# weiyithu/PV-RAFT

Hardware: AMD Instinct MI355X
Metric: train_pairs_per_sec (higher is better)
Workload: dtype bf16; 1 GPU; model=PV-RAFT (RSF stage 1), global_batch=2, points=8192, gru_iters=8, truncate_k=512, parallelism=dp1, hipgraph=True

## Files before the change

### pvraft_amd/csrc/bindings.cpp

```cpp
#include <torch/extension.h>
#include <ATen/hip/HIPContext.h>
#include <hip/hip_runtime.h>

#include <map>
#include <string>
#include <utility>

void launch_knn_graph(const float*, int*, int, int, int, hipStream_t);
void launch_knn_csr(const int*, int*, int*, int*, int*, int*, unsigned char*,
                    int, int, int, hipStream_t);
void launch_knn_interp(const float*, const float*, const float*, float*, int*,
                       float*, int, int, int, int, int, float, hipStream_t);
int knn_interp_tile_pts();
void launch_chamfer_fwd(const float*, const float*, const float*, float*, int*,
                        float*, int*, float*, int, int, int, int, int,
                        hipStream_t);
void launch_chamfer_bwd(const float*, const float*, const float*, const int*,
                        const int*, const float*, float*, int, int, int, int,
                        hipStream_t);
int chamfer_fwd_blocks(int, int, int);
int chamfer_tile_pts();
void launch_flow_smooth_fwd(const float*, const int*, float*, int, int, int,
                            int, hipStream_t);
void launch_flow_smooth_bwd(const float*, const int*, const int*, const int*,
// ... 1006 lines not shown
                                            std::vector<torch::Tensor> dbs) {
  const int n = (int)dys.size();
  TORCH_CHECK(n >= 1 && n <= 4095, "1..4095 jobs");
  TORCH_CHECK((int)xs.size() == n && (int)dws.size() == n && (int)dbs.size() == n);
  std::vector<PwWgradJob> jobs(n);
  long base_blocks = 0;
  const int TILE = 64;
  for (int j = 0; j < n; ++j) {
    auto& dy = dys[j];
    auto& x = xs[j];
    auto& dw = dws[j];
    TORCH_CHECK(dy.is_cuda() && dy.is_contiguous() && dy.dim() == 3 &&
                dy.scalar_type() == torch::kBFloat16, "dy must be (B,Co,S) bf16");
    TORCH_CHECK(x.is_cuda() && x.is_contiguous() && x.dim() == 3 &&
                x.scalar_type() == torch::kBFloat16, "x must be (B,Ci,S) bf16");
    TORCH_CHECK(dy.size(0) == x.size(0) && dy.size(2) == x.size(2), "dy/x mismatch");
    const bool dw_block = dw.dim() == 2 && !dw.is_contiguous();
    TORCH_CHECK(dw.is_cuda() && dw.scalar_type() == torch::kFloat32 &&
                (dw_block ? (dw.stride(1) == 1 && dw.stride(0) >= dw.size(1))
                          : dw.is_contiguous()),
                "dw must be fp32, contiguous or a row-contiguous block");
    const int Co = dy.size(1), Ci = x.size(1);
    TORCH_CHECK(dw.numel() == (long)Co * Ci &&
                (!dw_block || (dw.size(0) == Co && dw.size(1) == Ci)),
                "dw shape mismatch");
    const int ldw = dw_block ? (int)dw.stride(0) : Ci;
    TORCH_CHECK(Co <= 16 * TILE && Ci <= 16 * TILE, "Co/Ci too large for 4-bit tile index");
    float* dbias = nullptr;
    if (dbs[j].defined() && dbs[j].numel() > 0) {
      TORCH_CHECK(dbs[j].is_cuda() && dbs[j].is_contiguous() &&
                  dbs[j].scalar_type() == torch::kFloat32 && dbs[j].numel() == Co);
      dbias = dbs[j].data_ptr<float>();
    }
    jobs[j] = PwWgradJob{dy.data_ptr(), x.data_ptr(), dw.data_ptr<float>(),
                         dbias, Co, Ci, (int)dy.size(0), 1, dy.size(2), ldw,
                         0};
    base_blocks += (long)((Co + TILE - 1) / TILE) * ((Ci + TILE - 1) / TILE) *
                   dy.size(0);
  }
  (void)base_blocks;
  for (int j = 0; j < n; ++j) {
    long sc = (jobs[j].S + 3071) / 3072;
    if (sc < 1) sc = 1;
    if ((long)jobs[j].B * sc > 4095) sc = 4095 / jobs[j].B;
    jobs[j].schunks = (int)sc;
  }
  std::vector<unsigned int> map;
  map.reserve(4096);
  for (int j = 0; j < n; ++j) {
    const int to = (jobs[j].Co + TILE - 1) / TILE;
    const int ti = (jobs[j].Ci + TILE - 1) / TILE;
    const int bzs = jobs[j].B * jobs[j].schunks;
    for (int bz = 0; bz < bzs; ++bz)
      for (int a = 0; a < to; ++a)
        for (int b = 0; b < ti; ++b)
          map.push_back(((unsigned)j << 20) | ((unsigned)bz << 8) |
                        ((unsigned)a << 4) | (unsigned)b);
  }
  const long jbytes = (long)n * sizeof(PwWgradJob);
  const long mbytes = (long)map.size() * sizeof(unsigned int);
  std::vector<unsigned char> blob(jbytes + mbytes);
  memcpy(blob.data(), jobs.data(), jbytes);
  memcpy(blob.data() + jbytes, map.data(), mbytes);
  auto dev = torch::empty({jbytes + mbytes}, dys[0].options().dtype(torch::kUInt8));
  launch_desc_fill(dev.data_ptr(), blob.data(), jbytes + mbytes, stream());
  launch_pw_wgrad_batched(dev.data_ptr(),
                          (const unsigned int*)((char*)dev.data_ptr() + jbytes),
                          (int)map.size(), stream());
  return {dev};
}

torch::Tensor batched_transpose(torch::Tensor x) {
  TORCH_CHECK(x.is_cuda() && x.dim() == 3, "x must be 3-D GPU");
  TORCH_CHECK(x.stride(2) == 1 && x.stride(1) == x.size(2),
              "rows must be contiguous");
  const bool bf16 = x.scalar_type() == torch::kBFloat16;
  TORCH_CHECK(bf16 || x.scalar_type() == torch::kFloat32, "fp32/bf16 only");
  const int B = x.size(0);
  const long R = x.size(1), C = x.size(2);
  auto out = torch::empty({B, C, R}, x.options());
  launch_transpose(x.data_ptr(), out.data_ptr(), x.stride(0), B, R, C, bf16,
                   stream());
  return out;
}

std::vector<torch::Tensor> pv_corr_fused_fwd(torch::Tensor corr,
                                             torch::Tensor xyz,
                                             torch::Tensor coords,
                                             double base_scale,
                                             int64_t num_levels, int64_t k) {
  check_f32(corr, "corr");
  check_f32(xyz, "xyz");
  check_f32(coords, "coords");
  const int B = corr.size(0), N = corr.size(1), K = corr.size(2);
  TORCH_CHECK(K <= 512 && num_levels >= 1 && num_levels <= 4 && k >= 1 && k <= 64 && k <= K);
  auto vox = torch::empty({B, num_levels * 27, N}, corr.options());
  auto knn = torch::empty({B, 4, k, N}, corr.options());
  auto idx = torch::empty({B, N, k}, corr.options().dtype(torch::kInt32));
  launch_pv_corr_fused_fwd(corr.data_ptr<float>(), xyz.data_ptr<float>(),
                           coords.data_ptr<float>(), vox.data_ptr<float>(),
                           knn.data_ptr<float>(), idx.data_ptr<int>(), B, N, K,
                           (int)num_levels, (int)k, (float)base_scale, stream());
  return {vox, knn, idx};
}

torch::Tensor pv_corr_fused_bwd(torch::Tensor g_vox, torch::Tensor g_knn,
                                torch::Tensor xyz, torch::Tensor coords,
                                torch::Tensor knn_idx, int64_t num_levels,
                                int64_t k, double base_scale) {
  check_f32(g_vox, "g_vox");
  check_f32(g_knn, "g_knn");
  const int B = xyz.size(0), N = xyz.size(1), K = xyz.size(2);
  auto gcorr = torch::empty({B, N, K}, g_vox.options());
  launch_pv_corr_fused_bwd(g_vox.data_ptr<float>(), g_knn.data_ptr<float>(),
                           xyz.data_ptr<float>(), coords.data_ptr<float>(),
                           knn_idx.data_ptr<int>(), gcorr.data_ptr<float>(), B,
                           N, K, (int)num_levels, (int)k, (float)base_scale,
                           stream());
  return gcorr;
}

void launch_corr_topk(const void*, const void*, float*, float*, int*, float*,
                      int*, int*, int, int, int, int, int, float,
                      hipStream_t);

std::vector<torch::Tensor> corr_topk(torch::Tensor f1t, torch::Tensor f2t,
                                     int64_t K) {
  TORCH_CHECK(f1t.is_cuda() && f1t.is_contiguous() && f1t.dim() == 3 &&
              f1t.scalar_type() == torch::kBFloat16, "f1t must be (B,N,C) bf16");
  TORCH_CHECK(f2t.is_cuda() && f2t.is_contiguous() && f2t.dim() == 3 &&
              f2t.scalar_type() == torch::kBFloat16, "f2t must be (B,M,C) bf16");
  const int B = f1t.size(0), N = f1t.size(1), C = f1t.size(2);
  const int M = f2t.size(1);
  TORCH_CHECK(f2t.size(0) == B && f2t.size(2) == C, "f1t/f2t mismatch");
  TORCH_CHECK(C % 32 == 0 && C <= 256, "need C % 32 == 0, C <= 256");
  TORCH_CHECK(K >= 1 && K <= M && K <= 1024, "need 1 <= K <= min(M, 1024)");
  auto fopt = f1t.options().dtype(torch::kFloat32);
  auto iopt = f1t.options().dtype(torch::kInt32);
  const long R = (long)B * N;
  auto thr = torch::empty({R, 2}, fopt);
  auto out_v = torch::empty({B, (long)N, K}, fopt);
  auto out_i = torch::empty({B, (long)N, K}, iopt);
  auto band_v = torch::empty({R, 704}, fopt);
  auto band_i = torch::empty({R, 704}, iopt);
  auto cnt = zeros_fast({R, 2}, iopt);
  launch_corr_topk(f1t.data_ptr(), f2t.data_ptr(), thr.data_ptr<float>(),
                   out_v.data_ptr<float>(), out_i.data_ptr<int>(),
                   band_v.data_ptr<float>(), band_i.data_ptr<int>(),
                   cnt.data_ptr<int>(), B, N, M, C, (int)K,
                   1.0f / sqrtf((float)C), stream());
  return {out_v, out_i};
}

std::vector<torch::Tensor> topk_rows(torch::Tensor vals, int64_t K) {
  check_f32(vals, "vals");
  TORCH_CHECK(vals.dim() == 2, "vals must be (R, M)");
  const long R = vals.size(0);
  const int M = vals.size(1);
  TORCH_CHECK(M <= 8192, "topk_rows supports M <= 8192");
  TORCH_CHECK(K >= 1 && K <= M, "need 1 <= K <= M");
  auto out_v = torch::empty({R, K}, vals.options());
  auto out_i = torch::empty({R, K}, vals.options().dtype(torch::kInt32));
  launch_topk_rows(vals.data_ptr<float>(), out_v.data_ptr<float>(),
                   out_i.data_ptr<int>(), R, M, (int)K, stream());
  return {out_v, out_i};
}

namespace {

void check_gru(const torch::Tensor& t, const torch::Tensor& like,
               const char* name) {
  TORCH_CHECK(t.is_cuda() && t.is_contiguous(), name,
              " must be a contiguous GPU tensor");
  TORCH_CHECK(t.scalar_type() == like.scalar_type(), name,
              " dtype mismatch in fused GRU gates");
}

}

std::vector<torch::Tensor> gru_zr_fwd(torch::Tensor pre, torch::Tensor h) {
  TORCH_CHECK(pre.is_cuda() && pre.is_contiguous() && h.is_contiguous());
  TORCH_CHECK(pre.dim() == 3 && h.dim() == 3 && pre.size(0) == h.size(0) &&
              pre.size(1) == 2 * h.size(1) && pre.size(2) == h.size(2));
  const bool bf16 = pre.scalar_type() == torch::kBFloat16;
  TORCH_CHECK(bf16 || pre.scalar_type() == torch::kFloat32);
  check_gru(h, pre, "h");
  auto z = torch::empty_like(h), r = torch::empty_like(h),
       rh = torch::empty_like(h);
  launch_gru_zr_fwd(pre.data_ptr(), h.data_ptr(), z.data_ptr(), r.data_ptr(),
                    rh.data_ptr(), h.size(0), (long)h.size(1) * h.size(2),
                    bf16, stream());
  return {z, r, rh};
}

std::vector<torch::Tensor> gru_zr_bwd(torch::Tensor dz, torch::Tensor drh,
                                      torch::Tensor z, torch::Tensor r,
                                      torch::Tensor h) {
  const bool bf16 = z.scalar_type() == torch::kBFloat16;
  for (auto* t : {&dz, &drh, &r, &h}) check_gru(*t, z, "gru_zr_bwd input");
  auto dpre = torch::empty({h.size(0), 2 * h.size(1), h.size(2)}, h.options());
  auto dh = torch::empty_like(h);
  launch_gru_zr_bwd(dz.data_ptr(), drh.data_ptr(), z.data_ptr(), r.data_ptr(),
                    h.data_ptr(), dpre.data_ptr(), dh.data_ptr(), h.size(0),
                    (long)h.size(1) * h.size(2), bf16, stream());
  return {dpre, dh};
}

std::vector<torch::Tensor> gru_q_fwd(torch::Tensor pre, torch::Tensor z,
                                     torch::Tensor h) {
  const bool bf16 = pre.scalar_type() == torch::kBFloat16;
  TORCH_CHECK(bf16 || pre.scalar_type() == torch::kFloat32);
  for (auto* t : {&pre, &z, &h}) check_gru(*t, pre, "gru_q_fwd input");
  auto q = torch::empty_like(h), hnew = torch::empty_like(h);
  launch_gru_q_fwd(pre.data_ptr(), z.data_ptr(), h.data_ptr(), q.data_ptr(),
                   hnew.data_ptr(), h.size(0), (long)h.size(1) * h.size(2),
                   bf16, stream());
  return {q, hnew};
}

std::vector<torch::Tensor> gru_q_bwd(torch::Tensor dhnew, torch::Tensor q,
                                     torch::Tensor z, torch::Tensor h) {
  const bool bf16 = q.scalar_type() == torch::kBFloat16;
  for (auto* t : {&dhnew, &z, &h}) check_gru(*t, q, "gru_q_bwd input");
  auto dpre = torch::empty_like(h), dz = torch::empty_like(h),
       dh = torch::empty_like(h);
  launch_gru_q_bwd(dhnew.data_ptr(), q.data_ptr(), z.data_ptr(), h.data_ptr(),
                   dpre.data_ptr(), dz.data_ptr(), dh.data_ptr(), h.size(0),
                   (long)h.size(1) * h.size(2), bf16, stream());
  return {dpre, dz, dh};
}

std::vector<torch::Tensor> seq_loss_fwd(std::vector<torch::Tensor> flows,
                                        torch::Tensor gt, torch::Tensor mask,
                                        double gamma) {
  const int T = (int)flows.size();
  TORCH_CHECK(T >= 1 && T <= 32, "seq_loss supports 1..32 flows");
  check_f32(gt, "gt");
  check_f32(mask, "mask");
  const long BN = gt.numel() / 3;
  TORCH_CHECK(mask.numel() == BN, "mask/gt shape mismatch");
  const float* ptrs[32];
  for (int t = 0; t < T; ++t) {
    check_f32(flows[t], "flow");
    TORCH_CHECK(flows[t].numel() == BN * 3, "flow shape mismatch");
    ptrs[t] = flows[t].data_ptr<float>();
  }
  auto fopt = gt.options();
  static torch::Tensor* ws_p = new torch::Tensor();
  torch::Tensor& ws = *ws_p;
  if (!ws.defined()) ws = torch::zeros({33}, fopt);
  auto loss = torch::empty({}, fopt);
  auto denom = torch::empty({}, fopt);
  launch_seq_loss_fwd(ptrs, gt.data_ptr<float>(), mask.data_ptr<float>(),
                      ws.data_ptr<float>(), loss.data_ptr<float>(),
                      denom.data_ptr<float>(), BN, T, 1, (float)gamma,
                      stream());
  return {loss, denom};
}

std::vector<torch::Tensor> seq_loss_bwd(std::vector<torch::Tensor> flows,
                                        torch::Tensor gt, torch::Tensor mask,
                                        torch::Tensor dloss,
                                        torch::Tensor denom, double gamma) {
  const int T = (int)flows.size();
  TORCH_CHECK(T >= 1 && T <= 32);
  const long BN = gt.numel() / 3;
  const float* ptrs[32];
  float* gptrs[32];
  std::vector<torch::Tensor> grads;
  grads.reserve(T);
  for (int t = 0; t < T; ++t) {
    ptrs[t] = flows[t].data_ptr<float>();
    grads.push_back(torch::empty_like(flows[t]));
    gptrs[t] = grads[t].data_ptr<float>();
  }
  launch_seq_loss_bwd(ptrs, gptrs, gt.data_ptr<float>(),
                      mask.data_ptr<float>(), dloss.data_ptr<float>(),
                      denom.data_ptr<float>(), BN, T, 1, (float)gamma,
                      stream());
  return grads;
}

static void check_i32(const torch::Tensor& t, const char* name) {
  TORCH_CHECK(t.is_cuda() && t.is_contiguous() && t.scalar_type() == torch::kInt32,
              name, " must be a contiguous int32 GPU tensor");
}

static void chamfer_check(const torch::Tensor& pc1, const torch::Tensor& pc2,
                          int64_t T) {
  check_f32(pc1, "pc1");
  check_f32(pc2, "pc2");
  TORCH_CHECK(pc1.dim() == 3 && pc1.size(2) == 3, "pc1 must be (B,N,3)");
  TORCH_CHECK(pc2.dim() == 3 && pc2.size(2) == 3, "pc2 must be (B,M,3)");
  TORCH_CHECK(pc2.device() == pc1.device(), "chamfer inputs must share a device");
  const int64_t B = pc1.size(0), N = pc1.size(1), M = pc2.size(1);
  TORCH_CHECK(pc2.size(0) == B, "chamfer batch mismatch");
  TORCH_CHECK(T >= 1 && T <= 32, "chamfer supports 1..32 flows");
  TORCH_CHECK(B >= 1 && B <= 65535 && N >= 1 && M >= 1,
              "chamfer requires 1 <= B <= 65535, N, M >= 1");
  TORCH_CHECK(N < (1L << 31) - 256 && M < (1L << 31) - 256,
              "chamfer sizes exceed 32-bit point indexing");
}

std::vector<torch::Tensor> chamfer_fwd(torch::Tensor pc1, torch::Tensor flows,
                                       torch::Tensor pc2) {
  check_f32(flows, "flows");
// ... 206 lines not shown
  TORCH_CHECK(M >= 1 && M <= 256, "cluster_points requires 1 <= max_objects <= 256");
  TORCH_CHECK(min_points >= 3, "cluster_points requires min_points >= 3");
  TORCH_CHECK(eps >= 0.0 && flow_eps >= 0.0, "cluster_points requires eps, flow_eps >= 0");
  TORCH_CHECK(mask.is_cuda() && mask.is_contiguous() &&
                  mask.scalar_type() == torch::kBool && mask.dim() == 2 &&
                  mask.size(0) == B && mask.size(1) == N &&
                  mask.device() == xyz.device(),
              "mask must be contiguous bool (B,N) on the device of xyz");
  auto iopt = xyz.options().dtype(torch::kInt32);
  auto ws = torch::empty({5, B, N}, iopt);
  auto status = torch::empty({B}, iopt);
  auto labels = torch::empty({B, N}, iopt);
  auto count = torch::empty({B, M}, iopt);
  auto nobj = torch::empty({B}, iopt);
  launch_cluster_points(
      xyz.data_ptr<float>(), flow.data_ptr<float>(),
      reinterpret_cast<const unsigned char*>(mask.data_ptr<bool>()),
      ws.data_ptr<int>(), status.data_ptr<int>(), labels.data_ptr<int>(),
      count.data_ptr<int>(), nobj.data_ptr<int>(), (int)B, (int)N, (int)M,
      (float)eps, (float)flow_eps, (int)std::min<int64_t>(min_points, INT32_MAX),
      stream());
  return {labels, count, nobj};
}

std::vector<torch::Tensor> plane_fit(torch::Tensor xyz,
                                     c10::optional<torch::Tensor> mask,
                                     double thresh, double thresh2, double cos2,
                                     double upx, double upy, double upz,
                                     int64_t H, int64_t refine_iters,
                                     int64_t seed) {
  check_f32(xyz, "xyz");
  TORCH_CHECK(xyz.dim() == 3 && xyz.size(2) == 3, "xyz must be (B,N,3)");
  const int64_t B = xyz.size(0), N = xyz.size(1);
  TORCH_CHECK(B >= 1 && B <= 65535 && N >= 1, "plane_fit requires 1 <= B <= 65535, N >= 1");
  TORCH_CHECK(N < (1L << 30), "plane_fit sizes exceed 32-bit point indexing");
  TORCH_CHECK(H >= 1 && H <= 4096, "plane_fit requires 1 <= hypotheses <= 4096");
  TORCH_CHECK(refine_iters <= 16, "plane_fit requires refine_iters <= 16");
  TORCH_CHECK(thresh > 0.0 && thresh2 > 0.0, "plane_fit requires thresh > 0");
  const unsigned char* mp = nullptr;
  if (mask.has_value()) {
    const torch::Tensor& m = *mask;
    TORCH_CHECK(m.is_cuda() && m.is_contiguous() &&
                    m.scalar_type() == torch::kBool && m.dim() == 2 &&
                    m.size(0) == B && m.size(1) == N &&
                    m.device() == xyz.device(),
                "mask must be contiguous bool (B,N) on the device of xyz");
    mp = reinterpret_cast<const unsigned char*>(m.data_ptr<bool>());
  }
  auto iopt = xyz.options().dtype(torch::kInt32);
  auto bopt = xyz.options().dtype(torch::kBool);
  auto idx = torch::empty({B, H, 3}, iopt);
  auto cnt = torch::empty({B, H}, iopt);
  auto rec = torch::empty({B, H, 8}, xyz.options());
  launch_plane_hypotheses(xyz.data_ptr<float>(), mp, idx.data_ptr<int>(),
                          rec.data_ptr<float>(), cnt.data_ptr<int>(), (int)B,
                          (int)N, (int)H, (unsigned)(seed & 0xffffffffL),
                          (float)upx, (float)upy, (float)upz, (float)cos2,
                          (float)thresh2, stream());
  if (refine_iters < 0) return {idx, cnt};
  auto normal = torch::empty({B, 3}, xyz.options());
  auto offset = torch::empty({B}, xyz.options());
  auto height = torch::empty({B, N}, xyz.options());
  auto ground = torch::empty({B, N}, bopt);
  auto inlier = torch::empty({B, N}, bopt);
  auto count = torch::empty({B}, iopt);
  auto best = torch::empty({B}, iopt);
  auto rounds = torch::empty({B}, iopt);
  auto ok = torch::empty({B}, bopt);
  auto plane64 = torch::empty({B, 8}, xyz.options().dtype(torch::kFloat64));
  launch_plane_refine(
      xyz.data_ptr<float>(), mp, rec.data_ptr<float>(), cnt.data_ptr<int>(),
      normal.data_ptr<float>(), offset.data_ptr<float>(),
      height.data_ptr<float>(),
      reinterpret_cast<unsigned char*>(ground.data_ptr<bool>()),
      reinterpret_cast<unsigned char*>(inlier.data_ptr<bool>()),
      count.data_ptr<int>(), best.data_ptr<int>(), rounds.data_ptr<int>(),
      reinterpret_cast<unsigned char*>(ok.data_ptr<bool>()),
      plane64.data_ptr<double>(), (int)B, (int)N, (int)H, (int)refine_iters,
      thresh, (float)upx, (float)upy, (float)upz, (float)cos2, stream());
  return {normal, offset, height, ground, inlier, count, best, rounds, ok};
}

std::vector<torch::Tensor> voxel_sample(torch::Tensor xyz,
                                        c10::optional<torch::Tensor> mask,
                                        int64_t m, double inv, int64_t levels,
                                        int64_t seed) {
  check_f32(xyz, "xyz");
  TORCH_CHECK(xyz.dim() == 3 && xyz.size(2) == 3, "xyz must be (B,N,3)");
  const int64_t B = xyz.size(0), N = xyz.size(1);
  TORCH_CHECK(B >= 1 && B <= 65535 && N >= 1, "voxel_sample requires 1 <= B <= 65535, N >= 1");
  TORCH_CHECK(N < (1L << 27), "voxel_sample requires N < 2^27");
  TORCH_CHECK(m >= 1, "voxel_sample requires m >= 1");
  TORCH_CHECK(levels >= 1 && levels <= 16, "voxel_sample requires 1 <= levels <= 16");
  TORCH_CHECK(inv > 0.0 && std::isfinite(inv), "voxel_sample requires a finite 1 / voxel > 0");
  const unsigned char* mp = nullptr;
  if (mask.has_value()) {
    const torch::Tensor& k = *mask;
    TORCH_CHECK(k.is_cuda() && k.is_contiguous() &&
                    k.scalar_type() == torch::kBool && k.dim() == 2 &&
                    k.size(0) == B && k.size(1) == N &&
                    k.device() == xyz.device(),
                "mask must be contiguous bool (B,N) on the device of xyz");
    mp = reinterpret_cast<const unsigned char*>(k.data_ptr<bool>());
  }
  int64_t T = 2;
  while (T < 2 * N) T <<= 1;
  const int64_t nblk = (N + voxel_sample_block() - 1) / voxel_sample_block();
  auto iopt = xyz.options().dtype(torch::kInt32);
  auto lopt = xyz.options().dtype(torch::kInt64);
  auto tab = torch::empty({6, B, T}, lopt);
  auto key0 = torch::empty({B, N}, lopt);
  auto slots = torch::empty({2, B, N}, iopt);
  auto sel = torch::empty({B, N}, xyz.options().dtype(torch::kUInt8));
  auto bsum = torch::empty({B, nblk}, iopt);
  auto meta = torch::empty({B, (int64_t)voxel_sample_meta()}, iopt);
  auto idx = torch::empty({B, m}, lopt);
  auto count = torch::empty({B}, iopt);
  auto rank = torch::empty({B, N}, iopt);
  auto occ = torch::empty({B, levels}, iopt);
  launch_voxel_sample(
      xyz.data_ptr<float>(), mp,
      reinterpret_cast<unsigned long long*>(tab.data_ptr<int64_t>()),
      reinterpret_cast<unsigned long long*>(key0.data_ptr<int64_t>()),
      slots.data_ptr<int>(), sel.data_ptr<uint8_t>(), bsum.data_ptr<int>(),
      meta.data_ptr<int>(), reinterpret_cast<long*>(idx.data_ptr<int64_t>()),
      count.data_ptr<int>(), rank.data_ptr<int>(), occ.data_ptr<int>(), (int)B,
      (int)N, (int)T, (long)m, (int)levels, (float)inv,
      (unsigned)(seed & 0xffffffffL), stream());
  return {idx, count, rank, occ};
}

PYBIND11_MODULE(TORCH_EXTENSION_NAME, m) {
  m.def("voxel_sample", &voxel_sample);
  m.attr("VOXEL_SAMPLE_BLOCK") = voxel_sample_block();
  m.attr("VOXEL_SAMPLE_SCAN") = voxel_sample_scan();
  m.def("plane_fit", &plane_fit);
  m.attr("PLANE_SCORE_TILE") = plane_score_tile();
  m.attr("PLANE_SCORE_BLOCK") = plane_score_block();
  m.attr("PLANE_REFINE_BLOCK") = plane_refine_block();
  m.def("rigid_fit", &rigid_fit);
  m.attr("RIGID_FIT_REG_POINTS") = rigid_fit_reg_points();
  m.def("segmented_rigid_fit", &segmented_rigid_fit);
  m.attr("SEGMENTED_FIT_CAPACITY") = segmented_fit_capacity();
  m.def("cluster_points", &cluster_points);
  m.attr("CLUSTER_TILE") = cluster_tile();
  m.def("chamfer_fwd", &chamfer_fwd);
  m.def("chamfer_nn_fwd", &chamfer_nn_fwd);
  m.def("chamfer_bwd", &chamfer_bwd);
  m.attr("CHAMFER_TILE") = chamfer_tile_pts();
  m.def("flow_smooth_fwd", &flow_smooth_fwd);
  m.def("flow_smooth_bwd", &flow_smooth_bwd);
  m.def("topk_rows", &topk_rows);
  m.def("corr_topk", &corr_topk);
  m.def("seq_loss_fwd", &seq_loss_fwd);
  m.def("seq_loss_bwd", &seq_loss_bwd);
  m.def("gru_zr_fwd", &gru_zr_fwd);
  m.def("gru_zr_bwd", &gru_zr_bwd);
  m.def("gru_q_fwd", &gru_q_fwd);
  m.def("gru_q_bwd", &gru_q_bwd);
  m.def("pv_corr_fused_fwd", &pv_corr_fused_fwd);
  m.def("pv_corr_fused_bwd", &pv_corr_fused_bwd);
  m.def("pw_wgrad", &pw_wgrad, pybind11::arg("dy"), pybind11::arg("x"), pybind11::arg("schunks") = 0, pybind11::arg("with_bias") = false);
  m.def("pw_wgrad_batched", &pw_wgrad_batched);
  m.def("pw_fwd", &pw_fwd, pybind11::arg("ws"), pybind11::arg("xs"),
        pybind11::arg("bias"), pybind11::arg("addend"), pybind11::arg("act"),
        pybind11::arg("point_major") = false);
  m.def("pw_bwd", &pw_bwd, pybind11::arg("dy"), pybind11::arg("y"),
        pybind11::arg("ws"), pybind11::arg("want"), pybind11::arg("act"),
        pybind11::arg("point_major") = false,
        pybind11::arg("slab") = pybind11::none(), pybind11::arg("r0") = 0);
  m.def("batched_transpose", &batched_transpose);
  m.def("group_norm_act_fwd", &group_norm_act_fwd);
  m.def("group_norm_act_bwd", &group_norm_act_bwd);
  m.def("group_norm_act_maxpool_fwd", &group_norm_act_maxpool_fwd);
  m.def("group_norm_act_maxpool_bwd", &group_norm_act_maxpool_bwd);
  m.def("edge_gnmp_fwd", &edge_gnmp_fwd, pybind11::arg("wg"),
        pybind11::arg("idx"), pybind11::arg("G"), pybind11::arg("weight"),
        pybind11::arg("bias"), pybind11::arg("eps"), pybind11::arg("act"),
        pybind11::arg("slope"), pybind11::arg("slope_t"),
        pybind11::arg("channel_major_out") = false,
        pybind11::arg("classic") = false);
  m.def("edge_gnmp_bwd", &edge_gnmp_bwd, pybind11::arg("dy"),
        pybind11::arg("wg"), pybind11::arg("idx"), pybind11::arg("am"),
        pybind11::arg("vsel"), pybind11::arg("vsum"),
        pybind11::arg("offsets"), pybind11::arg("order_n"),
        pybind11::arg("order_j"), pybind11::arg("mean"),
        pybind11::arg("rstd"), pybind11::arg("G"), pybind11::arg("weight"),
        pybind11::arg("bias"), pybind11::arg("act"), pybind11::arg("slope"),
        pybind11::arg("slope_t"), pybind11::arg("wtarget"),
        pybind11::arg("btarget"), pybind11::arg("starget"),
        pybind11::arg("classic") = false);
  m.def("morton_keys", &morton_keys);
  m.def("multi_cast_bf16", &multi_cast_bf16);
  m.def("knn_gnmp_fwd", &knn_gnmp_fwd, pybind11::arg("raw"),
        pybind11::arg("W"), pybind11::arg("cb"), pybind11::arg("G"),
        pybind11::arg("gamma"), pybind11::arg("beta"), pybind11::arg("eps"),
        pybind11::arg("slope_t"), pybind11::arg("out_bf16"),
        pybind11::arg("channel_major_out") = false);
  m.def("knn_gnmp_bwd", &knn_gnmp_bwd, pybind11::arg("dy"),
        pybind11::arg("raw"), pybind11::arg("W"), pybind11::arg("cb"),
        pybind11::arg("am"), pybind11::arg("vsel"), pybind11::arg("mean"),
        pybind11::arg("rstd"), pybind11::arg("G"), pybind11::arg("gamma"),
        pybind11::arg("beta"), pybind11::arg("slope_t"), pybind11::arg("eps"),
        pybind11::arg("dy_channel_major") = false,
        pybind11::arg("wtarget") = pybind11::none(),
        pybind11::arg("cbtarget") = pybind11::none(),
        pybind11::arg("gtarget") = pybind11::none(),
        pybind11::arg("btarget") = pybind11::none(),
        pybind11::arg("starget") = pybind11::none());
  m.def("knn_graph", &knn_graph, "fused kNN graph (CDNA4)");
  m.def("knn_csr", &knn_csr, "inverse kNN adjacency as CSR (counting sort)");
  m.def("knn_interp_fwd", &knn_interp_fwd);
  m.attr("KNN_INTERP_TILE") = knn_interp_tile_pts();
  m.def("gather_edge_concat_fwd", &gather_edge_concat_fwd);
  m.def("gather_edge_concat_bwd", &gather_edge_concat_bwd);
  m.def("gather_edge_bwd_csr", &gather_edge_bwd_csr);
  m.def("voxel_corr_fwd", &voxel_corr_fwd);
  m.def("voxel_corr_bwd", &voxel_corr_bwd);
  m.def("knn_corr_fwd", &knn_corr_fwd);
  m.def("knn_corr_bwd", &knn_corr_bwd);
}
```

### pvraft_amd/model/corr.py

```python

from __future__ import annotations

from dataclasses import dataclass

import torch
import torch.nn as nn
from torch import Tensor

from pvraft_amd import ops
from .norm import FusedGroupNorm, PReLUAny
from .pointwise import PwConv1d, PwConv2d


@dataclass
class CorrField:
    corr: Tensor
    xyz: Tensor


class CorrBlock(nn.Module):
    def __init__(
        self,
        num_levels: int = 3,
        base_scale: float = 0.25,
        resolution: int = 3,
        truncate_k: int = 512,
        knn: int = 32,
    ):
        super().__init__()
        self.truncate_k = truncate_k
        self.num_levels = num_levels
        self.resolution = resolution
        self.base_scale = base_scale
        self.knn = knn
        self.out_conv = nn.Sequential(
            PwConv1d((resolution ** 3) * num_levels, 128, 1),
            FusedGroupNorm(8, 128),
            PReLUAny(),
            PwConv1d(128, 64, 1),
        )
        self.knn_conv = nn.Sequential(
            PwConv2d(4, 64, 1),
            FusedGroupNorm(8, 64),
            PReLUAny(),
        )
        self.knn_out = PwConv1d(64, 64, 1)

    def build(self, fmap1: Tensor, fmap2: Tensor, xyz2: Tensor) -> CorrField:
        corr, _idx, txyz = ops.corr_truncate(fmap1, fmap2, xyz2, self.truncate_k)
        return CorrField(corr=corr, xyz=txyz)

    def forward(self, field: CorrField, coords: Tensor) -> Tensor:
        vox, knn_raw = ops.pv_corr_lookup(
            field.corr, field.xyz, coords, self.base_scale, self.num_levels,
            self.knn, self.resolution,
        )
        return self._voxel_conv(vox) + self._knn_conv(knn_raw)

    def _voxel_feature(self, field: CorrField, coords: Tensor) -> Tensor:
        feat = ops.voxel_corr(
            field.corr, field.xyz, coords, self.base_scale, self.num_levels, self.resolution
        )
        return self._voxel_conv(feat)

    def _voxel_conv(self, feat: Tensor) -> Tensor:
        conv1, gn, prelu, conv2 = self.out_conv[0], self.out_conv[1], self.out_conv[2], self.out_conv[3]
        x = conv1(feat)
        x = ops.group_norm_act(
            x, gn.num_groups, gn.weight, gn.bias, gn.eps, act="prelu", slope_t=prelu.weight
        )
        return conv2(x)

    def _knn_feature(self, field: CorrField, coords: Tensor) -> Tensor:
        feat = ops.knn_corr(field.corr, field.xyz, coords, self.knn)
        return self._knn_conv(feat)

    def _knn_conv(self, feat: Tensor) -> Tensor:
        conv, gn, prelu = self.knn_conv[0], self.knn_conv[1], self.knn_conv[2]
        import os

        if (
            feat.is_cuda
            and ops.hip_available()
            and feat.dtype == torch.float32
            and conv.out_channels % 16 == 0
            and os.environ.get("PVRAFT_REF_OPS", "0") != "1"
            and os.environ.get("PVRAFT_NO_KNN_GNMP", "0") != "1"
        ):
            feat = ops.knn_gnmp(
                feat, conv.weight, conv.bias, gn.num_groups, gn.weight,
                gn.bias, gn.eps, prelu.weight,
            )
        else:
            feat = conv(feat)
            feat = ops.group_norm_act_maxpool(
                feat, gn.num_groups, gn.weight, gn.bias, gn.eps, act="prelu",
                slope_t=prelu.weight,
            )
        return self.knn_out(feat)
```

### pvraft_amd/ops/__init__.py

```python

from __future__ import annotations

import math
import os
from typing import NamedTuple, Optional, Tuple

import torch
from torch import Tensor

from . import reference

_EXT = None
_EXT_ERR: Optional[str] = None


def _load_ext():
    global _EXT, _EXT_ERR
    if _EXT is None and _EXT_ERR is None:
        try:
            from pvraft_amd import _C

            _EXT = _C
        except ImportError as e:
            _EXT_ERR = str(e)
# ... 351 lines not shown
        if pointwise._DEFER.on and all(
            p.is_leaf and p.requires_grad for p in params
        ):
            bufs = [pointwise._grad_buffer(p) for p in params]
            if all(t.dtype == torch.float32 and t.is_contiguous()
                   for t in bufs):
                (draw,) = _EXT.knn_gnmp_bwd(
                    dy, raw, w, cb, am, vsel, mean, rstd, num_groups, ga,
                    be, st, eps, cm, *[t.view(-1) for t in bufs])
            else:
                draw, *grads = _EXT.knn_gnmp_bwd(
                    dy, raw, w, cb, am, vsel, mean, rstd, num_groups, ga,
                    be, st, eps, cm)
                for t, g in zip(bufs, grads):
                    t.view(-1).add_(g.view(-1))
            return (draw, None, None, None, None, None, None, None, None)
        draw, dW, dcb, dgamma, dbeta, dslope = _EXT.knn_gnmp_bwd(
            dy, raw, w, cb, am, vsel, mean, rstd, num_groups, ga, be, st, eps,
            cm)
        return (draw, dW.view(wshape).to(wdtype), dcb, None, dgamma, dbeta,
                None, dslope.reshape(1), None)


def knn_gnmp(raw: Tensor, weight: Tensor, cbias: Tensor, num_groups: int,
             gamma: Tensor, beta: Tensor, eps: float, slope_t: Tensor,
             channel_major_out: Optional[bool] = None) -> Tensor:
    if not _use_hip(raw):
        raise RuntimeError("knn_gnmp is a GPU-only fused op")
    if channel_major_out is None:
        channel_major_out = channel_major_layout()
    if channel_major_out:
        return _KnnGNMP.apply(raw.contiguous(), weight, cbias, num_groups,
                              gamma, beta, eps, slope_t, True)
    y = _KnnGNMP.apply(raw.contiguous(), weight, cbias, num_groups, gamma,
                       beta, eps, slope_t)
    return transpose_last2(y)




_ARANGE_CACHE: dict = {}


def morton_order(xyz: Tensor, need_inv: bool = True):
    if not _use_hip(xyz):
        raise RuntimeError("morton_order is a GPU-only op")
    mn, mx = torch.aminmax(xyz, dim=1)
    mn = mn.contiguous()
    inv_ext = (1023.0 / (mx - mn).clamp_min(1e-9)).contiguous()
    keys = _EXT.morton_keys(xyz.contiguous(), mn, inv_ext)
    perm = keys.argsort(dim=1)
    inv = None
    if need_inv:
        B, N = perm.shape
        ck = (B, N, xyz.device.index)
        ar = _ARANGE_CACHE.get(ck)
        if ar is None:
            ar = torch.arange(N, device=xyz.device).expand(B, N).contiguous()
            _ARANGE_CACHE[ck] = ar
        inv = torch.empty_like(perm)
        inv.scatter_(1, perm, ar)
    return perm, inv


def knn_graph_pair(xyz: Tensor, k: int) -> Tuple[Tensor, Optional[Tensor]]:
    xyz = xyz.contiguous().float()
    if _use_hip(xyz):
        idx32 = _EXT.knn_graph(xyz, k)
        return idx32.long(), idx32
    return reference.knn_idx(xyz, k), None


def knn_graph(xyz: Tensor, k: int) -> Tensor:
    return knn_graph_pair(xyz, k)[0]


def knn_csr(idx32: Tensor) -> Tuple[Tensor, Tensor, Tensor, Tensor]:
    if _load_ext() is None:
        raise RuntimeError(f"pvraft_amd._C is not built: {_EXT_ERR}")
    return tuple(_EXT.knn_csr(idx32.contiguous()))


class _KnnInterpolate(torch.autograd.Function):

    @staticmethod
    def forward(ctx, support_xyz, values, query_xyz, k, eps):
        out, idx32, w = _EXT.knn_interp_fwd(support_xyz, values, query_xyz, k, eps)
        idx = idx32.long()
        ctx.save_for_backward(idx, w)
        ctx.n_support = values.shape[1]
        ctx.mark_non_differentiable(idx, w)
        return out, idx, w

    @staticmethod
    def backward(ctx, dout, _didx, _dw):
        idx, w = ctx.saved_tensors
        B, M, ke = idx.shape
        C = dout.shape[2]
        rows = (idx.clamp_min(0) + torch.arange(B, device=idx.device).view(B, 1, 1) * ctx.n_support).reshape(-1)
        contrib = (w.unsqueeze(-1) * dout.unsqueeze(2)).reshape(B * M * ke, C)
        dvalues = torch.zeros(B * ctx.n_support, C, dtype=dout.dtype, device=dout.device)
        dvalues.index_add_(0, rows, contrib)
        return None, dvalues.view(B, ctx.n_support, C), None, None, None


def knn_interpolate(
    support_xyz: Tensor, values: Tensor, query_xyz: Tensor, k: int = 3, eps: float = 1e-8
) -> Tuple[Tensor, Tensor, Tensor]:
    if not 1 <= int(k) <= 16:
        raise ValueError(f"knn_interpolate requires 1 <= k <= 16, got {k}")
    if _use_hip(support_xyz):
        return _KnnInterpolate.apply(
            support_xyz.detach().float().contiguous(),
            values.float().contiguous(),
            query_xyz.detach().float().contiguous(),
            int(k),
            float(eps),
        )
    if not (support_xyz.dtype == values.dtype == query_xyz.dtype == torch.float64):
        support_xyz, values, query_xyz = support_xyz.float(), values.float(), query_xyz.float()
    return reference.knn_interpolate(
        support_xyz.detach().contiguous(), values.contiguous(), query_xyz.detach().contiguous(), int(k), float(eps)
    )


def gather_edge_concat(feats: Tensor, idx: Tensor, xyz: Tensor, csr=None) -> Tensor:
    if not feats.is_contiguous():
        if (
            feats.is_cuda
            and feats.dim() == 3
            and feats.stride(1) == 1
            and feats.stride(2) == feats.shape[1]
            and feats.dtype in (torch.float32, torch.bfloat16)
            and os.environ.get("PVRAFT_REF_OPS", "0") != "1"
            and _load_ext() is not None
        ):
            feats = _BatchedTranspose.apply(feats.transpose(1, 2))
        else:
            feats = feats.contiguous()
    if _use_hip(feats):
        if feats.dtype not in (torch.float32, torch.bfloat16):
            feats = feats.float()
        order, offsets = (csr[0], csr[1]) if csr is not None else (None, None)
        return _GatherEdgeConcat.apply(
            feats, idx.to(torch.int32).contiguous(), xyz.contiguous().float(),
            order, offsets,
        )
    return reference.gather_edge_concat(feats, idx, xyz)


class _CorrTruncate(torch.autograd.Function):

    CHUNK = 2048

    @staticmethod
    def forward(ctx, fmap1: Tensor, fmap2: Tensor, xyz2: Tensor, truncate_k: int):
        with torch.no_grad(), torch.autocast("cuda", enabled=False):
            M = fmap2.shape[2]
            if (
                fmap1.is_cuda
                and fmap1.dtype == torch.bfloat16
                and fmap2.dtype == torch.bfloat16
                and fmap1.shape[1] % 32 == 0
                and fmap1.shape[1] <= 256
                and truncate_k <= 1024
                and _load_ext() is not None
            ):
                K = min(truncate_k, M)
                f1t = _EXT.batched_transpose(fmap1.contiguous())
                f2t = _EXT.batched_transpose(fmap2.contiguous())
                corr, idx32 = _EXT.corr_topk(f1t, f2t, K)
                idx = idx32.long()
                B, _, N = fmap1.shape
                txyz = xyz2.gather(
                    1, idx.reshape(B, N * K).unsqueeze(-1).expand(B, N * K, 3)
                ).view(B, N, K, 3)
            elif fmap1.is_cuda and M <= 8192 and _load_ext() is not None:
                corr, idx, txyz = _CorrTruncate._gpu_forward(
                    fmap1.float(), fmap2.float(), xyz2, truncate_k
                )
            else:
                corr, idx, txyz = reference.corr_truncate(
                    fmap1.float(), fmap2.float(), xyz2, truncate_k,
                    chunk=_CorrTruncate.CHUNK,
                )
        ctx.save_for_backward(fmap1, fmap2, idx)
        ctx.bf16_bwd = fmap1.is_cuda and (
            torch.is_autocast_enabled() or fmap1.dtype == torch.bfloat16
        )
        return corr, idx, txyz

    @staticmethod
    def _gpu_forward(fmap1: Tensor, fmap2: Tensor, xyz2: Tensor, truncate_k: int):
        B, C, N = fmap1.shape
        M = fmap2.shape[2]
        K = min(truncate_k, M)
        scale = 1.0 / math.sqrt(C)
        f1t = fmap1.transpose(1, 2).contiguous()
        chunk = _CorrTruncate.CHUNK
        vals, idxs = [], []
        for s in range(0, N, chunk):
            c = torch.bmm(f1t[:, s : s + chunk], fmap2)
            c = c * scale
            n_rows = c.shape[1]
            v, i = _EXT.topk_rows(c.reshape(B * n_rows, M), K)
            vals.append(v.view(B, n_rows, K))
            idxs.append(i.view(B, n_rows, K).long())
        corr = torch.cat(vals, dim=1)
        idx = torch.cat(idxs, dim=1)
        txyz = xyz2.gather(1, idx.reshape(B, N * K).unsqueeze(-1).expand(B, N * K, 3)).view(B, N, K, 3)
        return corr, idx, txyz

    @staticmethod
    def backward(ctx, g_corr: Tensor, _g_idx, _g_xyz):
        fmap1, fmap2, idx = ctx.saved_tensors
        B, C, N = fmap1.shape
        M = fmap2.shape[2]
        scale = 1.0 / math.sqrt(C)
        dt = torch.bfloat16 if ctx.bf16_bwd else g_corr.dtype
        gfull = torch.zeros(B, N, M, dtype=dt, device=g_corr.device)
        gfull.scatter_(2, idx, (g_corr * scale).to(dt))
        f1 = fmap1.to(dt)
        f2 = fmap2.to(dt)
        if gfull.is_cuda and _load_ext() is not None:
            gfull_t = _EXT.batched_transpose(gfull)
        else:
            gfull_t = gfull.transpose(1, 2).contiguous()
        g1 = torch.bmm(f2, gfull_t).float()
        g2 = torch.bmm(f1, gfull).float()
        return g1, g2, None, None


def corr_truncate(fmap1: Tensor, fmap2: Tensor, xyz2: Tensor, truncate_k: int):
    if fmap1.is_cuda and os.environ.get("PVRAFT_REF_OPS", "0") != "1":
        return _CorrTruncate.apply(fmap1, fmap2, xyz2, truncate_k)
    return reference.corr_truncate(fmap1.float(), fmap2.float(), xyz2, truncate_k)


def voxel_corr(
    corr: Tensor,
    xyz: Tensor,
    coords: Tensor,
    base_scale: float,
    num_levels: int,
    resolution: int = 3,
) -> Tensor:
    if _use_hip(corr):
        return _VoxelCorr.apply(
            corr.contiguous().float(),
            xyz.contiguous().float(),
            coords.contiguous().float(),
            float(base_scale),
            int(num_levels),
            int(resolution),
        )
    return reference.voxel_corr(corr, xyz, coords, base_scale, num_levels, resolution)


class _PVCorrFused(torch.autograd.Function):

    @staticmethod
    def forward(ctx, corr, xyz, coords, base_scale, num_levels, k):
        vox, knn, idx = _EXT.pv_corr_fused_fwd(corr, xyz, coords, base_scale, num_levels, k)
        ctx.save_for_backward(xyz, coords, idx)
        ctx.conf = (base_scale, num_levels, k)
        return vox, knn

    @staticmethod
    def backward(ctx, g_vox, g_knn):
        xyz, coords, idx = ctx.saved_tensors
        base_scale, num_levels, k = ctx.conf
        g = _EXT.pv_corr_fused_bwd(
            g_vox.contiguous(), g_knn.contiguous(), xyz, coords, idx, num_levels, k, base_scale
        )
        return g, None, None, None, None, None


def pv_corr_lookup(
    corr: Tensor,
    xyz: Tensor,
    coords: Tensor,
    base_scale: float,
    num_levels: int,
    k: int,
    resolution: int = 3,
):
    if _use_hip(corr) and resolution == 3:
        return _PVCorrFused.apply(
            corr.contiguous().float(),
            xyz.contiguous().float(),
            coords.contiguous().float(),
            float(base_scale),
            int(num_levels),
            int(k),
        )
    return (
        reference.voxel_corr(corr, xyz, coords, base_scale, num_levels, resolution),
        reference.knn_corr(corr, xyz, coords, k),
    )


def knn_corr(corr: Tensor, xyz: Tensor, coords: Tensor, k: int) -> Tensor:
    if _use_hip(corr):
        return _KnnCorr.apply(
            corr.contiguous().float(),
            xyz.contiguous().float(),
            coords.contiguous().float(),
            int(k),
        )
    return reference.knn_corr(corr, xyz, coords, k)


class _GruZR(torch.autograd.Function):

    @staticmethod
    def forward(ctx, pre: Tensor, h: Tensor):
        z, r, rh = _EXT.gru_zr_fwd(pre, h)
        ctx.save_for_backward(z, r, h)
        return z, rh

    @staticmethod
    def backward(ctx, dz: Tensor, drh: Tensor):
        z, r, h = ctx.saved_tensors
        if dz is None:
            dz = torch.zeros_like(z)
        if drh is None:
            drh = torch.zeros_like(z)
        dpre, dh = _EXT.gru_zr_bwd(dz.contiguous(), drh.contiguous(), z, r, h)
        return dpre, dh


class _GruQ(torch.autograd.Function):

    @staticmethod
    def forward(ctx, pre: Tensor, z: Tensor, h: Tensor) -> Tensor:
        q, hnew = _EXT.gru_q_fwd(pre, z, h)
        ctx.save_for_backward(q, z, h)
        return hnew

    @staticmethod
    def backward(ctx, dhnew: Tensor):
        q, z, h = ctx.saved_tensors
        dpre, dz, dh = _EXT.gru_q_bwd(dhnew.contiguous(), q, z, h)
        return dpre, dz, dh


def gru_zr(pre_zr: Tensor, h: Tensor):
    if _use_hip(pre_zr) and os.environ.get("PVRAFT_NO_GRU_FUSION", "0") != "1":
        return _GruZR.apply(pre_zr.contiguous(), h.to(pre_zr.dtype).contiguous())
    hd = h.shape[1]
    zr = torch.sigmoid(pre_zr)
    return zr[:, :hd], zr[:, hd:] * h


def gru_q(pre_q: Tensor, z: Tensor, h: Tensor) -> Tensor:
    if _use_hip(pre_q) and os.environ.get("PVRAFT_NO_GRU_FUSION", "0") != "1":
        return _GruQ.apply(
            pre_q.contiguous(), z.contiguous(), h.to(pre_q.dtype).contiguous()
        )
    return (1 - z) * h + z * torch.tanh(pre_q)




class _ChamferLoss(torch.autograd.Function):

    @staticmethod
    def forward(ctx, pc1, flows, pc2):
        cham, _d1, i1, _d2, i2 = _EXT.chamfer_fwd(pc1, flows, pc2)
        ctx.save_for_backward(pc1, flows, pc2, i1, i2)
        return cham

    @staticmethod
    def backward(ctx, g):
        pc1, flows, pc2, i1, i2 = ctx.saved_tensors
        return None, _EXT.chamfer_bwd(pc1, flows, pc2, i1, i2, g.float().contiguous()), None


class _FlowSmoothness(torch.autograd.Function):

    @staticmethod
    def forward(ctx, flows, idx32, offsets, order_n):
        ctx.save_for_backward(flows, idx32, offsets, order_n)
        return _EXT.flow_smooth_fwd(flows, idx32)

    @staticmethod
    def backward(ctx, g):
        flows, idx32, offsets, order_n = ctx.saved_tensors
# ... 268 lines not shown
```

### setup.py

```python

import os

os.environ.setdefault("PYTORCH_ROCM_ARCH", "gfx950")

from setuptools import setup
from torch.utils.cpp_extension import BuildExtension, CUDAExtension

SOURCES = [
    "pvraft_amd/csrc/bindings.cpp",
    "pvraft_amd/csrc/knn_graph.hip",
    "pvraft_amd/csrc/knn_csr.hip",
    "pvraft_amd/csrc/knn_interp.hip",
    "pvraft_amd/csrc/gather_edge.hip",
    "pvraft_amd/csrc/voxel_corr.hip",
    "pvraft_amd/csrc/knn_corr.hip",
    "pvraft_amd/csrc/group_norm.hip",
    "pvraft_amd/csrc/edge_gnmp.hip",
    "pvraft_amd/csrc/knn_gnmp.hip",
    "pvraft_amd/csrc/cast_pack.hip",
    "pvraft_amd/csrc/pw_wgrad.hip",
    "pvraft_amd/csrc/pw_fwd.hip",
    "pvraft_amd/csrc/pw_bwd.hip",
    "pvraft_amd/csrc/transpose.hip",
    "pvraft_amd/csrc/pv_corr_fused.hip",
    "pvraft_amd/csrc/topk_rows.hip",
    "pvraft_amd/csrc/corr_topk.hip",
    "pvraft_amd/csrc/gru_gates.hip",
    "pvraft_amd/csrc/seq_loss.hip",
    "pvraft_amd/csrc/chamfer.hip",
    "pvraft_amd/csrc/flow_smooth.hip",
    "pvraft_amd/csrc/rigid_fit.hip",
    "pvraft_amd/csrc/cluster.hip",
    "pvraft_amd/csrc/plane_fit.hip",
    "pvraft_amd/csrc/voxel_sample.hip",
]

setup(
    name="pvraft_amd",
    version="0.1.0",
    packages=["pvraft_amd"],
    ext_modules=[
        CUDAExtension(
            name="pvraft_amd._C",
            sources=SOURCES,
            extra_compile_args={
                "cxx": ["-O3", "-std=c++17"],
                "nvcc": ["-O3", "-std=c++17", "--offload-arch=gfx950"],
            },
        )
    ],
    cmdclass={"build_ext": BuildExtension},
)
```

Baseline: 206.3 pairs/s.

## Fuse correlation gradient scatter into dense-row expand kernel and gather xyz natively

Replaces the zeros+scatter+transpose sequence in the truncated-correlation backward with one kernel. Each block builds a full gradient row in shared memory and streams it out. The following bmm then reads a transposed view instead of an explicitly transposed copy. It also adds a custom int32 xyz gather kernel to avoid the int64 index conversion and torch.gather in the forward, keeping indices int32 in the model path. The risks are limited occupancy from the 64 KB shared row image and a possibly slower bmm on the non-contiguous transposed operand.

```diff
diff --git a/pvraft_amd/csrc/bindings.cpp b/pvraft_amd/csrc/bindings.cpp
--- a/pvraft_amd/csrc/bindings.cpp
+++ b/pvraft_amd/csrc/bindings.cpp
@@ -1182,6 +1182,50 @@
   return {out_v, out_i};
 }
 
+void launch_corr_grad_expand(const float*, const int*, void*, long, int, int,
+                             float, bool, hipStream_t);
+void launch_corr_gather_xyz(const int*, const float*, float*, int, long, int,
+                            hipStream_t);
+
+torch::Tensor corr_grad_expand(torch::Tensor g, torch::Tensor idx,
+                               double scale, int64_t M, bool bf16) {
+  check_f32(g, "g");
+  TORCH_CHECK(g.dim() == 3, "g must be (B, N, K)");
+  TORCH_CHECK(idx.is_cuda() && idx.is_contiguous() &&
+              idx.scalar_type() == torch::kInt32 && idx.sizes() == g.sizes(),
+              "idx must be contiguous int32 of g's shape");
+  TORCH_CHECK(idx.device() == g.device(), "g and idx on different devices");
+  TORCH_CHECK(M >= 1 && M * (bf16 ? 2 : 4) <= 64 * 1024,
+              "row image limited to 64 KB");
+  const long B = g.size(0), N = g.size(1);
+  TORCH_CHECK(B * N < (1L << 31), "too many rows");
+  auto out = torch::empty(
+      {B, N, M}, g.options().dtype(bf16 ? torch::kBFloat16 : torch::kFloat32));
+  launch_corr_grad_expand(g.data_ptr<float>(), idx.data_ptr<int>(),
+                          out.data_ptr(), B * N, (int)g.size(2), (int)M,
+                          (float)scale, bf16, stream());
+  return out;
+}
+
+torch::Tensor corr_gather_xyz(torch::Tensor idx, torch::Tensor xyz2) {
+  check_f32(xyz2, "xyz2");
+  TORCH_CHECK(idx.is_cuda() && idx.is_contiguous() && idx.dim() == 3 &&
+              idx.scalar_type() == torch::kInt32,
+              "idx must be contiguous (B, N, K) int32");
+  TORCH_CHECK(xyz2.dim() == 3 && xyz2.size(2) == 3 &&
+              xyz2.size(0) == idx.size(0) && xyz2.size(1) >= 1,
+              "xyz2 must be (B, M, 3)");
+  TORCH_CHECK(idx.device() == xyz2.device(),
+              "idx and xyz2 on different devices");
+  const long B = idx.size(0), N = idx.size(1), K = idx.size(2);
+  TORCH_CHECK((B * N * K + 1023) / 1024 < (1L << 31), "too many entries");
+  auto out = torch::empty({B, N, K, 3}, xyz2.options());
+  launch_corr_gather_xyz(idx.data_ptr<int>(), xyz2.data_ptr<float>(),
+                         out.data_ptr<float>(), (int)B, N * K,
+                         (int)xyz2.size(1), stream());
+  return out;
+}
+
 std::vector<torch::Tensor> topk_rows(torch::Tensor vals, int64_t K) {
   check_f32(vals, "vals");
   TORCH_CHECK(vals.dim() == 2, "vals must be (R, M)");
@@ -1694,6 +1738,8 @@
   m.def("flow_smooth_bwd", &flow_smooth_bwd);
   m.def("topk_rows", &topk_rows);
   m.def("corr_topk", &corr_topk);
+  m.def("corr_grad_expand", &corr_grad_expand);
+  m.def("corr_gather_xyz", &corr_gather_xyz);
   m.def("seq_loss_fwd", &seq_loss_fwd);
   m.def("seq_loss_bwd", &seq_loss_bwd);
   m.def("gru_zr_fwd", &gru_zr_fwd);
diff --git a/pvraft_amd/csrc/corr_bwd.hip b/pvraft_amd/csrc/corr_bwd.hip
--- /dev/null
+++ b/pvraft_amd/csrc/corr_bwd.hip
@@ -0,0 +1,144 @@
+#include <hip/hip_runtime.h>
+#include <hip/hip_bf16.h>
+#include "common.h"
+
+#define CB_THREADS 256
+
+DEV_INLINE unsigned short cb_bf16_rne(float v) {
+  const unsigned u = __float_as_uint(v);
+  if (v != v) return 0x7FC0;
+  return (unsigned short)((u + 0x7FFFu + ((u >> 16) & 1u)) >> 16);
+}
+
+template <typename T>
+DEV_INLINE T cb_cvt(float v);
+template <>
+DEV_INLINE float cb_cvt<float>(float v) { return v; }
+template <>
+DEV_INLINE unsigned short cb_cvt<unsigned short>(float v) {
+  return cb_bf16_rne(v);
+}
+
+template <typename V>
+DEV_INLINE void cb_stream_row(const void *img, void *dst, int bytes) {
+  const V *s = (const V *)img;
+  V *d = (V *)dst;
+  const int n = bytes / (int)sizeof(V);
+  for (int i = threadIdx.x; i < n; i += CB_THREADS) d[i] = s[i];
+}
+
+template <typename T>
+__global__ __launch_bounds__(CB_THREADS) void corr_grad_expand_kernel(
+    const float *__restrict__ g,
+    const int *__restrict__ idx,
+    T *__restrict__ out,
+    int K, int M, float scale) {
+  extern __shared__ uint4 cb_img[];
+  T *img = (T *)cb_img;
+  const long r = blockIdx.x;
+  const int row_bytes = M * (int)sizeof(T);
+  const int nvec = (row_bytes + 15) >> 4;
+  for (int i = threadIdx.x; i < nvec; i += CB_THREADS)
+    cb_img[i] = make_uint4(0u, 0u, 0u, 0u);
+  __syncthreads();
+
+  const float *gr = g + r * K;
+  const int *ir = idx + r * K;
+  if ((K & 3) == 0 &&
+      (((unsigned long long)g | (unsigned long long)idx) & 15) == 0) {
+    for (int k = threadIdx.x * 4; k < K; k += CB_THREADS * 4) {
+      const float4 gv = *(const float4 *)(gr + k);
+      const int4 iv = *(const int4 *)(ir + k);
+      if ((unsigned)iv.x < (unsigned)M) img[iv.x] = cb_cvt<T>(gv.x * scale);
+      if ((unsigned)iv.y < (unsigned)M) img[iv.y] = cb_cvt<T>(gv.y * scale);
+      if ((unsigned)iv.z < (unsigned)M) img[iv.z] = cb_cvt<T>(gv.z * scale);
+      if ((unsigned)iv.w < (unsigned)M) img[iv.w] = cb_cvt<T>(gv.w * scale);
+    }
+  } else {
+    for (int k = threadIdx.x; k < K; k += CB_THREADS) {
+      const int m = ir[k];
+      if ((unsigned)m < (unsigned)M) img[m] = cb_cvt<T>(gr[k] * scale);
+    }
+  }
+  __syncthreads();
+
+  T *dst = out + r * M;
+  if ((row_bytes & 15) == 0) cb_stream_row<uint4>(img, dst, row_bytes);
+  else if ((row_bytes & 7) == 0) cb_stream_row<uint2>(img, dst, row_bytes);
+  else if ((row_bytes & 3) == 0) cb_stream_row<unsigned>(img, dst, row_bytes);
+  else cb_stream_row<T>(img, dst, row_bytes);
+}
+
+void launch_corr_grad_expand(const float *g, const int *idx, void *out,
+                             long rows, int K, int M, float scale, bool bf16,
+                             hipStream_t stream) {
+  if (rows <= 0) return;
+  const size_t esz = bf16 ? 2 : 4;
+  const size_t shmem = (((size_t)M * esz + 15) / 16) * 16;
+  if (bf16)
+    hipLaunchKernelGGL(corr_grad_expand_kernel<unsigned short>,
+                       dim3((unsigned)rows), dim3(CB_THREADS), shmem, stream,
+                       g, idx, (unsigned short *)out, K, M, scale);
+  else
+    hipLaunchKernelGGL(corr_grad_expand_kernel<float>, dim3((unsigned)rows),
+                       dim3(CB_THREADS), shmem, stream, g, idx, (float *)out,
+                       K, M, scale);
+}
+
+#define CG_EPT 4
+#define CG_TILE (CB_THREADS * CG_EPT)
+
+struct CgXyz { float x, y, z; };
+
+__global__ __launch_bounds__(CB_THREADS) void corr_gather_xyz_kernel(
+    const int *__restrict__ idx,
+    const float *__restrict__ xyz2,
+    float *__restrict__ out,
+    long total, long NK, int M) {
+  __shared__ __attribute__((aligned(16))) float tile[CG_TILE * 3];
+  const long e0 = (long)blockIdx.x * CG_TILE;
+  const long e = e0 + (long)threadIdx.x * CG_EPT;
+  if (e < total) {
+    int m[CG_EPT];
+    if (e + CG_EPT <= total && ((unsigned long long)idx & 15) == 0) {
+      const int4 iv = *(const int4 *)(idx + e);
+      m[0] = iv.x; m[1] = iv.y; m[2] = iv.z; m[3] = iv.w;
+    } else {
+#pragma unroll
+      for (int j = 0; j < CG_EPT; ++j) m[j] = (e + j < total) ? idx[e + j] : 0;
+    }
+    long b = e / NK;
+    long bend = (b + 1) * NK;
+#pragma unroll
+    for (int j = 0; j < CG_EPT; ++j) {
+      if (e + j >= bend) { ++b; bend += NK; }
+      const int mm = min(max(m[j], 0), M - 1);
+      const CgXyz p = (e + j < total)
+          ? *(const CgXyz *)(xyz2 + (b * M + mm) * 3) : CgXyz{0.f, 0.f, 0.f};
+      float *t = tile + (threadIdx.x * CG_EPT + j) * 3;
+      t[0] = p.x; t[1] = p.y; t[2] = p.z;
+    }
+  }
+  __syncthreads();
+  const long f0 = e0 * 3;
+  const long fend = total * 3;
+  for (int i = threadIdx.x * 4; i < CG_TILE * 3; i += CB_THREADS * 4) {
+    const long f = f0 + i;
+    if (f + 4 <= fend) {
+      *(float4 *)(out + f) = *(const float4 *)(tile + i);
+    } else {
+      for (int j = 0; j < 4; ++j)
+        if (f + j < fend) out[f + j] = tile[i + j];
+    }
+  }
+}
+
+void launch_corr_gather_xyz(const int *idx, const float *xyz2, float *out,
+                            int B, long NK, int M, hipStream_t stream) {
+  const long total = (long)B * NK;
+  if (total <= 0) return;
+  const long blocks = (total + CG_TILE - 1) / CG_TILE;
+  hipLaunchKernelGGL(corr_gather_xyz_kernel, dim3((unsigned)blocks),
+                     dim3(CB_THREADS), 0, stream, idx, xyz2, out, total, NK,
+                     M);
+}
diff --git a/pvraft_amd/model/corr.py b/pvraft_amd/model/corr.py
--- a/pvraft_amd/model/corr.py
+++ b/pvraft_amd/model/corr.py
@@ -47,7 +47,9 @@
         self.knn_out = PwConv1d(64, 64, 1)
 
     def build(self, fmap1: Tensor, fmap2: Tensor, xyz2: Tensor) -> CorrField:
-        corr, _idx, txyz = ops.corr_truncate(fmap1, fmap2, xyz2, self.truncate_k)
+        corr, _idx, txyz = ops.corr_truncate(
+            fmap1, fmap2, xyz2, self.truncate_k, index_dtype=torch.int32
+        )
         return CorrField(corr=corr, xyz=txyz)
 
     def forward(self, field: CorrField, coords: Tensor) -> Tensor:
diff --git a/pvraft_amd/ops/__init__.py b/pvraft_amd/ops/__init__.py
--- a/pvraft_amd/ops/__init__.py
+++ b/pvraft_amd/ops/__init__.py
@@ -527,9 +527,12 @@
 class _CorrTruncate(torch.autograd.Function):
 
     CHUNK = 2048
-
-    @staticmethod
-    def forward(ctx, fmap1: Tensor, fmap2: Tensor, xyz2: Tensor, truncate_k: int):
+    EXPAND_ROW_BYTES = 64 * 1024
+
+    @staticmethod
+    def forward(ctx, fmap1: Tensor, fmap2: Tensor, xyz2: Tensor, truncate_k: int,
+                index_dtype: torch.dtype = torch.int64):
+        classic = corr_bwd_classic()
         with torch.no_grad(), torch.autocast("cuda", enabled=False):
             M = fmap2.shape[2]
             if (
@@ -544,12 +547,15 @@
                 K = min(truncate_k, M)
                 f1t = _EXT.batched_transpose(fmap1.contiguous())
                 f2t = _EXT.batched_transpose(fmap2.contiguous())
-                corr, idx32 = _EXT.corr_topk(f1t, f2t, K)
-                idx = idx32.long()
+                corr, idx = _EXT.corr_topk(f1t, f2t, K)
                 B, _, N = fmap1.shape
-                txyz = xyz2.gather(
-                    1, idx.reshape(B, N * K).unsqueeze(-1).expand(B, N * K, 3)
-                ).view(B, N, K, 3)
+                if classic or xyz2.dtype != torch.float32:
+                    idx = idx.long()
+                    txyz = xyz2.gather(
+                        1, idx.reshape(B, N * K).unsqueeze(-1).expand(B, N * K, 3)
+                    ).view(B, N, K, 3)
+                else:
+                    txyz = _EXT.corr_gather_xyz(idx, xyz2.contiguous())
             elif fmap1.is_cuda and M <= 8192 and _load_ext() is not None:
                 corr, idx, txyz = _CorrTruncate._gpu_forward(
                     fmap1.float(), fmap2.float(), xyz2, truncate_k
@@ -563,7 +569,8 @@
         ctx.bf16_bwd = fmap1.is_cuda and (
             torch.is_autocast_enabled() or fmap1.dtype == torch.bfloat16
         )
-        return corr, idx, txyz
+        idx_out = idx.long() if index_dtype == torch.int64 else idx
+        return corr, idx_out, txyz
 
     @staticmethod
     def _gpu_forward(fmap1: Tensor, fmap2: Tensor, xyz2: Tensor, truncate_k: int):
@@ -580,10 +587,14 @@
             n_rows = c.shape[1]
             v, i = _EXT.topk_rows(c.reshape(B * n_rows, M), K)
             vals.append(v.view(B, n_rows, K))
-            idxs.append(i.view(B, n_rows, K).long())
+            idxs.append(i.view(B, n_rows, K))
         corr = torch.cat(vals, dim=1)
         idx = torch.cat(idxs, dim=1)
-        txyz = xyz2.gather(1, idx.reshape(B, N * K).unsqueeze(-1).expand(B, N * K, 3)).view(B, N, K, 3)
+        if corr_bwd_classic() or xyz2.dtype != torch.float32:
+            idx = idx.long()
+            txyz = xyz2.gather(1, idx.reshape(B, N * K).unsqueeze(-1).expand(B, N * K, 3)).view(B, N, K, 3)
+        else:
+            txyz = _EXT.corr_gather_xyz(idx, xyz2.contiguous())
         return corr, idx, txyz
 
     @staticmethod
@@ -593,22 +604,41 @@
         M = fmap2.shape[2]
         scale = 1.0 / math.sqrt(C)
         dt = torch.bfloat16 if ctx.bf16_bwd else g_corr.dtype
-        gfull = torch.zeros(B, N, M, dtype=dt, device=g_corr.device)
-        gfull.scatter_(2, idx, (g_corr * scale).to(dt))
         f1 = fmap1.to(dt)
         f2 = fmap2.to(dt)
+        if (
+            g_corr.is_cuda
+            and not corr_bwd_classic()
+            and dt in (torch.bfloat16, torch.float32)
+            and M * dt.itemsize <= _CorrTruncate.EXPAND_ROW_BYTES
+            and _load_ext() is not None
+        ):
+            gfull = _EXT.corr_grad_expand(
+                g_corr.float().contiguous(), idx.to(torch.int32), scale, M,
+                dt == torch.bfloat16,
+            )
+            g1 = torch.bmm(f2, gfull.transpose(1, 2)).float()
+            g2 = torch.bmm(f1, gfull).float()
+            return g1, g2, None, None, None
+        gfull = torch.zeros(B, N, M, dtype=dt, device=g_corr.device)
+        gfull.scatter_(2, idx.long(), (g_corr * scale).to(dt))
         if gfull.is_cuda and _load_ext() is not None:
             gfull_t = _EXT.batched_transpose(gfull)
         else:
             gfull_t = gfull.transpose(1, 2).contiguous()
         g1 = torch.bmm(f2, gfull_t).float()
         g2 = torch.bmm(f1, gfull).float()
-        return g1, g2, None, None
-
-
-def corr_truncate(fmap1: Tensor, fmap2: Tensor, xyz2: Tensor, truncate_k: int):
+        return g1, g2, None, None, None
+
+
+def corr_bwd_classic() -> bool:
+    return os.environ.get("PVRAFT_CORR_BWD", "") == "classic"
+
+
+def corr_truncate(fmap1: Tensor, fmap2: Tensor, xyz2: Tensor, truncate_k: int,
+                  index_dtype: torch.dtype = torch.int64):
     if fmap1.is_cuda and os.environ.get("PVRAFT_REF_OPS", "0") != "1":
-        return _CorrTruncate.apply(fmap1, fmap2, xyz2, truncate_k)
+        return _CorrTruncate.apply(fmap1, fmap2, xyz2, truncate_k, index_dtype)
     return reference.corr_truncate(fmap1.float(), fmap2.float(), xyz2, truncate_k)
 
 
diff --git a/setup.py b/setup.py
--- a/setup.py
+++ b/setup.py
@@ -25,6 +25,7 @@
     "pvraft_amd/csrc/pv_corr_fused.hip",
     "pvraft_amd/csrc/topk_rows.hip",
     "pvraft_amd/csrc/corr_topk.hip",
+    "pvraft_amd/csrc/corr_bwd.hip",
     "pvraft_amd/csrc/gru_gates.hip",
     "pvraft_amd/csrc/seq_loss.hip",
     "pvraft_amd/csrc/chamfer.hip",
```

Result: faster. 214.7 pairs/s (median of 6 runs) (+4.1%).
